# eldar/deepcut-cnn

Measured on AMD Instinct MI355X. Metric: images/sec, DeeperCut ResNet-152 FCN forward (prob+loc_pred+next_pred), whole node, higher is better.
Workload: dtype f32

## Files before the change

deepcut-cnn_amd/csrc/kernels.h:

```cpp
#pragma once
#include <cstddef>
#include <cstdint>
#include <string>

namespace dc {

constexpr int kMaxTaps = 32;

void dc_magic(unsigned d, unsigned (&mg)[2]);

enum ElemKind { kElemF32 = 0, kElemF16 = 1, kElemBF16 = 2 };
inline int elem_kind_size(int kind) { return kind == kElemF32 ? 4 : 2; }
inline const char* elem_kind_name(int kind) { return kind == kElemF16 ? "f16" : kind == kElemBF16 ? "bf16" : "f32"; }

constexpr int kMaxClasses = 4;
struct ConvClass {
  int nty, ntx, dy0, ddy, x0, ddx, Ktot, x_bias;
  int OH, OW, M;
  int tiles_m;
  unsigned div_ohw[2];
  unsigned div_ow[2];
  long w_off;
  long y_off;
};
// ... 20 lines not shown
  int end[8][kMaxProblems];
  ConvProblem prob[kMaxProblems];
};

struct ConvGemmParams {
  int esize;
  const void* x;
  long x_img_stride;
  int x_row_stride;
  int x_rows;
  int x_rowlen;
  int sy, sx;
  int nty, ntx;
  int dy0, ddy;
  int x0, ddx;
  int klen;
  int x_bias;
  const void* w;
  int Ktot;
  int NB, OH, OW;
  int M;
  int Cout;
  void* y;
  long y_img_stride;
  int y_row_stride;
  int y_pix_stride;
  const void* resid;
  const float* scale;
  const float* shift;
  int relu;
  int sigmoid_ch;
  int xcd_on;
  int xcd_lgx;
  int tiles_m;
  unsigned div_rw[2][2];
  unsigned div_ohw[2];
  unsigned div_ow[2];
  unsigned div_tn[2];
  int tiles_n;
  long long* dbg;
  int w_TY, w_TX, w_NBY, w_NBX, w_nblk;
  unsigned w_div_nblk[2], w_div_nbyx[2], w_div_dd[2], w_div_d[2], w_div_nbx[2];
  int wide_epi;
  int vec_epi;
  int dense_x;
  int dense_y;
  int ncls;
  int mc_lgx;
  ConvClass cls[kMaxClasses];
  int nprob;
  int ekind;
};
struct ConvMultiArgs {
  ConvGemmParams p;
  ConvMultiTable t;
};
static_assert(sizeof(ConvMultiArgs) <= 4096, "HIP kernel arguments are limited to 4 KB");

struct ConvVariant {
  const char* name;
  int BM, BN, WR, WC, WK;
};
int conv_num_variants();
const ConvVariant& conv_variant(int i);
int conv_variant_bk(int i);
int conv_variant_esize(int i);
constexpr int kBf16Variant0 = 2000;
int conv_num_bf16_variants();
inline bool is_bf16_variant(int v) { return v >= kBf16Variant0 && v < kBf16Variant0 + conv_num_bf16_variants(); }
int conv_variant_ekind(int v);
bool conv_variant_exists(int v);
const int* conv_variants_of(int ekind, int* count);
int conv_variant_by_name(const char* name);
bool conv_variant_multiclass(int i);
long conv_grid(const ConvGemmParams& p, int variant);
int launch_conv_gemm(const ConvGemmParams& p, int variant, void* stream);
long prepare_conv_multi(ConvGemmParams& p, ConvMultiTable& table, int nprob, int variant);
bool conv_variant_multiproblem(int i);
int launch_conv_multi(const ConvMultiArgs& a, int variant, long grid, void* stream);

bool wino_eligible(const ConvGemmParams& p);
bool wino_same3x3(const ConvGemmParams& p);
ConvGemmParams wino_launch_params(const ConvGemmParams& p, long grid, int bty, int btx, int blocks_per_wg);
long wino_grid(const ConvGemmParams& p);
size_t wino_packed_floats(int Cout, int Cin);
void wino_pack_filters(const float* g, int Cout, int Cin, float* out);
bool wino_half_eligible(const ConvGemmParams& p);
long wino_half_grid(const ConvGemmParams& p);
size_t wino_half_packed_elems(int Cout, int Cin);
void wino_half_pack_filters(const float* g, int Cout, int Cin, bool rowscale, float* out, float* row_scale);
int launch_wino_half(const ConvGemmParams& p, void* stream);
bool stream1x1_eligible(const ConvGemmParams& p);
long stream1x1_grid(const ConvGemmParams& p);
size_t stream1x1_packed_elems(int Cout, int K);
void stream1x1_pack_filters(const float* g, int Cout, int K, float* out);
int launch_stream1x1(const ConvGemmParams& p, void* stream);
bool stream1x1f_eligible(const ConvGemmParams& p);
long stream1x1f_grid(const ConvGemmParams& p);
size_t stream1x1f_packed_elems(int Cout, int K);
void stream1x1f_pack_filters(const float* g, int Cout, int K, float* out);
int launch_stream1x1f(const ConvGemmParams& p, void* stream);
bool stem_ws_eligible(const ConvGemmParams& p);
long stem_ws_grid(const ConvGemmParams& p);
size_t stem_ws_packed_elems();
void stem_ws_pack_filters(const float* rowtap, float* out);
int launch_stem_ws(const ConvGemmParams& p, void* stream);
bool stem7x7_eligible(const ConvGemmParams& p);
long stem7x7_grid(const ConvGemmParams& p);
size_t stem7x7_packed_elems();
void stem7x7_pack_filters(const float* g, int C, float* out);
int launch_stem7x7(const ConvGemmParams& p, void* stream);
long stream1x1_prepare_multi(const ConvGemmParams& p, const ConvMultiTable& tb, int nprob);
int launch_stream1x1_multi(const ConvMultiArgs& a, void* stream);

constexpr int kWinoVariant = 1000;
constexpr int kWinoVariant16 = 1001;
constexpr int kWinoHalf = 1002;
constexpr int kStreamHalf = 1003;
constexpr int kStemHalf = 1004;
constexpr int kStreamFloat = 1005;
constexpr int kStemFloat = 1006;
constexpr int kFormVariant0 = kWinoVariant, kNumForms = 7;
enum FormGeometry { kForm3x3, kForm1x1, kFormStem };
struct ConvForm {
  int variant;
  const char *name, *label;
  int ekind, geometry, waves;
  const char* const* timing_slots;
  bool (*eligible)(const ConvGemmParams& p);
  long (*grid)(const ConvGemmParams& p);
  int (*launch)(const ConvGemmParams& p, void* stream);
  bool own_scale;
  bool merges;
  long (*prepare_multi)(const ConvGemmParams& p, const ConvMultiTable& tb, int nprob);
  int (*launch_multi)(const ConvMultiArgs& a, void* stream);
  int sibling;
  const char* env;
};
const ConvForm* conv_form(int variant);

const char* variant_name(int v);
int variant_by_name(const char* name);
std::string variant_kernel_label(int v);
long variant_grid(const ConvGemmParams& p, int v);
int launch_conv(const ConvGemmParams& p, int v, void* stream);


int launch_maxpool(const void* x, void* y, int ekind, int NB, int H, int W, int C, int OH, int OW, int k, int s,
                   int pad, void* stream);

int launch_eltwise(const void* x, const void* z, const float* a, const float* b, void* y, int ekind, long total, int C,
                   int relu, int sigmoid, void* stream);

int launch_crop(const void* x, void* y, int ekind, int NB, int H, int W, int C, int oh, int ow, int OH, int OW,
                void* stream);

int launch_nchw_to_nhwc(const float* src, void* dst, int ekind, int NB, int C, int H, int W, int CP, void* stream);
int launch_nhwc_to_nchw(const void* src, void* dst, int ekind, int NB, int C, int H, int W, int CP, int c0,
                        void* stream, int dst_esize = 4);
int launch_f32_to_f16(const float* src, void* dst, long n, void* stream);
int launch_f32_to_bf16(const float* src, void* dst, long n, void* stream);

int launch_part_select(const void* prob, int pcp, int pc0, const void* loc, int lcp, int lc0, int ekind, int NB, int H, int W, int J, float thr,
                       int radius, double scale, int max_det, unsigned long long* spill, int* counts, double* out, void* stream);
int launch_pairwise_decode(const void* next, int ncp, int nc0, int ekind, int NB, int H, int W, int E, double scale, int ndet,
                           const int* det , const double* mean, const double* stdev, double* out,
                           void* stream);

struct ImagePrepParams {
  const unsigned char* src;
  int n, h, w;
  int out_h, out_w;
  int use_h, use_w;
  const int* x_bounds;
  const int* x_coeffs;
  int x_ksize;
  const int* y_bounds;
  const int* y_coeffs;
  int y_ksize;
  unsigned char* tmp;
  int row0, rows;
  void* dst;
  int dst_ekind, dst_cp;
  float mean[3];
};
int launch_image_prep(const ImagePrepParams& p, void* stream);

struct BoxPrepItem {
  int x0, y0, h, w;
  int use_h, use_w;
  const int* x_bounds;
  const int* x_coeffs;
  const int* y_bounds;
  const int* y_coeffs;
  int x_ksize, y_ksize;
};
struct BoxPrepParams {
  const unsigned char* src;
  int img_h, img_w;
  int n;
  int out_h, out_w;
  const BoxPrepItem* items;
  void* dst;
  int dst_ekind, dst_cp;
  float mean[3];
};
int launch_box_prep(const BoxPrepParams& p, void* stream);

int launch_pose_decode(const void* prob, int pcp, int pc0, const void* loc, int lcp, int lc0, int ekind, int NB, int H,
                       int W, int J, double scale, double* out, void* stream);
struct PoseDecodeItem {
  double scale, dx, dy;
  int rows, cols;
};
int launch_pose_decode_items(const void* prob, int pcp, int pc0, const void* loc, int lcp, int lc0, int ekind, int NB, int H,
                             int W, int J, const PoseDecodeItem* items, double* out, void* stream);

}
```

deepcut-cnn_amd/csrc/kernels.hip:

```cpp
#include <hip/hip_runtime.h>

#include <algorithm>
#include <cstdlib>
#include <cstring>
#include <type_traits>
#include <vector>

#include "kernel_prims.h"
#include "kernels.h"

namespace dc {


#define DC_KARG_TOUCH(n0, n1, n2, n3, n4)                                                                                  \
  unsigned n0, n1, n2, n3, n4;                                                                                             \
  {                                                                                                                        \
    const auto* ka_ = __builtin_amdgcn_kernarg_segment_ptr();                                                              \
    asm volatile("s_load_dword %0, %5, 0x0\n\ts_load_dword %1, %5, 0x40\n\ts_load_dword %2, %5, 0x80\n\ts_load_dword %3, %5, 0xc0\n\t" \
                 "s_load_dword %4, %5, 0x100"                                                                              \
                 : "=&s"(n0), "=&s"(n1), "=&s"(n2), "=&s"(n3), "=&s"(n4)                                                     \
                 : "s"(ka_));                                                                                              \
  }
#define DC_KARG_HOLD(n0, n1, n2, n3, n4) asm volatile("" ::"s"(n0), "s"(n1), "s"(n2), "s"(n3), "s"(n4))
static_assert(sizeof(ConvGemmParams) >= 0x140, "DC_KARG_TOUCH reads five 64-byte lines of the argument block");
// ... 1221 lines not shown
    const long g = f->prepare_multi ? f->prepare_multi(p, tb, nprob) : -1;
    if (g > 0) p.nprob = nprob, p.ncls = 0;
    return g;
  }
  if (!dc_variant_ok(variant) || nprob < 1 || nprob > kMaxProblems) return -1;
  const VariantEntry& e = entry_of(variant);
  if (!e.kernel_mp || p.esize != e.esize || (p.ekind == kElemBF16) != is_bf16_variant(variant) || p.klen % e.BK != 0) return -1;
  const long es = p.esize;
  const long tn = (p.Cout + e.v.BN - 1) / e.v.BN;
  bool vec = true;
  double atot = 0;
  long w_lo = 0, w_hi = 0;
  int rows[kMaxProblems];
  for (int c = 0; c < nprob; ++c) {
    ConvProblem& q = tb.prob[c];
    const int ntaps = q.nty * q.ntx;
    if (ntaps < 1 || ntaps > kMaxTaps || q.Ktot != ntaps * p.klen || q.M <= 0 || q.NB <= 0) return -1;
    if (!images_fit(es, q.NB, q.x_img_stride, q.y_img_stride)) return -1;
    if ((q.resid != nullptr) != (tb.prob[0].resid != nullptr)) return -1;
    q.x_bias = tap_bias(q, q.x_row_stride);
    set_m_tiles(q, e.v.BM);
    rows[c] = q.tiles_m;
    q.dense_x = dense_x_of(q, p);
    q.dense_y = dense_y_of(q);
    vec = vec && out_vec16(q, es);
    w_lo = std::min(w_lo, q.w_off);
    w_hi = std::max(w_hi, q.w_off + (long)p.Cout * q.Ktot);
    atot += (double)es * q.M * (double)p.klen * q.nty;
  }
  const double wtot = (double)es * (double)(w_hi - w_lo);
  if (wtot >= k2GiB) return -1;
  p.nprob = nprob;
  p.ncls = 0;
  set_epi(p, vec);
  p.dense_x = p.dense_y = 0;
  p.xcd_on = 0;
  p.tiles_n = (int)tn;
  dc_magic((unsigned)tn, p.div_tn);
  const long blk = mc_xcd_grid(p, rows, nprob, tn, wtot, atot);
  if (blk <= 0 || blk > 0x7fffffffL) return -1;
  {
    const int lgx = p.mc_lgx, lgy = 3 - lgx;
    const unsigned w0 = (unsigned)(tn >> lgx);
    dc_magic(std::max(w0, 1u), p.div_rw[0]);
    dc_magic(w0 + 1, p.div_rw[1]);
    for (int qy = 0; qy < 8; ++qy) {
      int run = 0;
      for (int c = 0; c < kMaxProblems; ++c) {
        if (c < nprob && qy < (8 >> lgx)) {
          run += (int)((((long)tb.prob[c].tiles_m * (qy + 1)) >> lgy) - (((long)tb.prob[c].tiles_m * qy) >> lgy));
          tb.end[qy][c] = run;
        } else {
          tb.end[qy][c] = 0x7fffffff;
        }
      }
    }
  }
  return blk;
}

int launch_conv_multi(const ConvMultiArgs& a, int variant, long grid, void* stream) {
  if (const ConvForm* f = conv_form(variant)) return f->launch_multi ? f->launch_multi(a, stream) : (int)hipErrorInvalidValue;
  if (!dc_variant_ok(variant) || !entry_of(variant).kernel_mp || a.p.nprob < 1 || grid <= 0) return (int)hipErrorInvalidValue;
  const VariantEntry& e = entry_of(variant);
  const int nt = e.v.WR * e.v.WC * e.v.WK * 64;
  hipLaunchKernelGGL(e.kernel_mp, dim3((unsigned)grid), dim3(nt), 0, (hipStream_t)stream, a);
  return (int)hipGetLastError();
}

namespace {
constexpr int WBTY = 4, WBTX = 8, WBN = 16, WKC = 32;
constexpr int WRH = 2 * WBTY + 2, WRW = 2 * WBTX + 2;
constexpr int WPSTR = WKC + 4;
constexpr int WPITCH = 672;
constexpr int WSTAGE = WRH * WPITCH + 8;
constexpr int WNTH = 512;
static_assert(WPITCH >= WRW * WPSTR && (2 * WPITCH) % 64 == 0 && WPSTR == 36, "conflict-free ds_read_b128 layout (see above)");
static_assert(WPITCH % 4 == 0 && WPSTR % 4 == 0 && WSTAGE % 4 == 0, "16-byte units");
__device__ __forceinline__ int wino_rowbase(int row) { return row * WPITCH; }
__device__ __forceinline__ f32x2 wlo(f32x4 v) { return __builtin_shufflevector(v, v, 0, 1); }
__device__ __forceinline__ f32x2 whi(f32x4 v) { return __builtin_shufflevector(v, v, 2, 3); }
}

template <int NG>
__global__ __launch_bounds__(WNTH * NG, 4) void wino_f23_kernel(const ConvGemmParams p) {
  constexpr int NTH = WNTH * NG;
  constexpr int WNLD = (WRH * WRW * (WKC / 4) + NTH - 1) / NTH;
  const long long t_entry = (long long)__builtin_amdgcn_s_memrealtime();
  DC_KARG_TOUCH(ka0, ka1, ka2, ka3, ka4);
  __shared__ __attribute__((aligned(16))) float stage[3][WSTAGE];
  float (*part)[4][2][2][4][64] = reinterpret_cast<float (*)[4][2][2][4][64]>(&stage[0][0]);
  static_assert(sizeof(float) * NG * 4 * 2 * 2 * 4 * 64 <= sizeof(stage), "partials must fit in the staging ring");
  static_assert(2 * sizeof(stage) <= 160 * 1024, "two workgroups per CU");
  const int t = threadIdx.x, lane = t & 63, wave = t >> 6;
  auto stamp = [&](int slot) {
    if (p.dbg && lane == 0) {
      long long* d = p.dbg + ((long)blockIdx.x * (8 * NG) + wave) * 12;
      d[slot] = (long long)__builtin_readcyclecounter();
      if (slot == 0) d[8] = t_entry, d[10] = (long long)__builtin_amdgcn_s_memrealtime();
      if (slot == 7) d[9] = (long long)__builtin_amdgcn_s_memrealtime();
    }
  };
  stamp(0);
  const int C = p.klen, H = p.x_rows, W = p.x_rowlen / p.klen;
  const int d = p.ddy;
  const int NBY = p.w_NBY, NBX = p.w_NBX;
  const int nblk = p.w_nblk;
  int lb = blockIdx.x;
  if (p.xcd_on) {
    const int g8 = gridDim.x >> 3, r8 = gridDim.x & 7, q = blockIdx.x & 7;
    lb = q * g8 + min(q, r8) + (blockIdx.x >> 3);
  }
  const int nt = dc_fastdiv(lb, p.w_div_nblk), blk = lb - nt * nblk;
  const int nph = dc_fastdiv(blk, p.w_div_nbyx), brem = blk - nph * (NBY * NBX);
  const int n = dc_fastdiv(nph, p.w_div_dd), ph = nph - n * (d * d);
  const int phy = dc_fastdiv(ph, p.w_div_d), phx = ph - phy * d;
  const int by = dc_fastdiv(brem, p.w_div_nbx), bx = brem - by * NBX;
  const int oy0 = 2 * WBTY * by - 1, ox0 = 2 * WBTX * bx - 1;
  DC_KARG_HOLD(ka0, ka1, ka2, ka3, ka4);
  const int kg = lane >> 4;
  const int grp = NG == 1 ? 0 : __builtin_amdgcn_readfirstlane(wave >> 3);
  const int i = wave & 3, tf = (wave >> 2) & 1;
  const int ra = i == 0 ? 0 : (i == 2 ? 2 : 1), rb = i == 0 ? 2 : (i == 1 ? 2 : (i == 2 ? 1 : 3));
  const float sb = i == 1 ? 1.f : -1.f;
  const __amdgpu_buffer_rsrc_t xr = dc_rsrc(reinterpret_cast<const float*>(p.x) + (long)n * p.x_img_stride, 0x7fffffffu);
  const __amdgpu_buffer_rsrc_t ur = dc_rsrc(p.w, 0x7fffffffu);
  unsigned gofs[WNLD];
  int sofs[WNLD];
#pragma unroll
  for (int q = 0; q < WNLD; ++q) {
    const int e = t + q * NTH;
    const int pix = e / (WKC / 4), cq = e % (WKC / 4);
    const int py = pix / WRW, px = pix % WRW;
    const int iy = phy + d * (oy0 + py), ix = phx + d * (ox0 + px);
    const bool ok = pix < WRH * WRW && oy0 + py >= 0 && ox0 + px >= 0 && iy < H && ix < W;
    gofs[q] = ok ? (unsigned)(iy * p.x_row_stride + ix * C + cq * 4) * 4u : kOOB;
    sofs[q] = (pix < WRH * WRW ? wino_rowbase(py) + px * WPSTR + cq * 4 : WSTAGE - 8 + (t & 1) * 4) >> 2;
  }
  const int r = (lane & 15) >> 3, c = lane & 7;
  const int ofs_a = wino_rowbase(2 * (2 * tf + r) + ra) + 2 * c * WPSTR + kg * 4;
  const int ofs_b = wino_rowbase(2 * (2 * tf + r) + rb) + 2 * c * WPSTR + kg * 4;
  f32x4 acc[4];
#pragma unroll
  for (int j = 0; j < 4; ++j) acc[j] = f32x4{0.f, 0.f, 0.f, 0.f};
  const unsigned uvo = ((unsigned)((nt * 4 + i) * (C / 16)) * (4 * 64 * 4) + (unsigned)lane * 4u) * 4u;
  f32x4 g[WNLD], b[2][4], da[4], db[4];
  auto gload = [&](int K) {
#pragma unroll
    for (int q = 0; q < WNLD; ++q) g[q] = dc_bload4(xr, gofs[q], (unsigned)(K * WKC * 4));
  };
  auto sstore = [&](int buf) {
#pragma unroll
    for (int q = 0; q < WNLD; ++q) reinterpret_cast<f32x4*>(&stage[buf][0])[sofs[q]] = g[q];
  };
  auto bload = [&](int slot, int k16) {
#pragma unroll
    for (int j = 0; j < 4; ++j) b[slot][j] = dc_bload4(ur, uvo + (unsigned)j * 1024u, (unsigned)k16 * 4096u);
  };
  auto lread = [&](int buf, int h) {
#pragma unroll
    for (int c4 = 0; c4 < 4; ++c4) {
      da[c4] = *reinterpret_cast<const f32x4*>(&stage[buf][ofs_a + c4 * WPSTR + h * 16]);
      db[c4] = *reinterpret_cast<const f32x4*>(&stage[buf][ofs_b + c4 * WPSTR + h * 16]);
    }
  };
  auto compute = [&](int bslot) {
    f32x2 tl[4], th[4];
    const f32x2 sb2 = {sb, sb};
#pragma unroll
    for (int c4 = 0; c4 < 4; ++c4) {
      tl[c4] = wlo(da[c4]) + sb2 * wlo(db[c4]);
      th[c4] = whi(da[c4]) + sb2 * whi(db[c4]);
    }
    f32x2 vl[4], vh[4];
    vl[0] = tl[0] - tl[2], vh[0] = th[0] - th[2];
    vl[1] = tl[1] + tl[2], vh[1] = th[1] + th[2];
    vl[2] = tl[2] - tl[1], vh[2] = th[2] - th[1];
    vl[3] = tl[1] - tl[3], vh[3] = th[1] - th[3];
#pragma unroll
    for (int j = 0; j < 4; ++j) acc[j] = __builtin_amdgcn_mfma_f32_16x16x4f32(vl[j][0], b[bslot][j][0], acc[j], 0, 0, 0);
#pragma unroll
    for (int j = 0; j < 4; ++j) acc[j] = __builtin_amdgcn_mfma_f32_16x16x4f32(vl[j][1], b[bslot][j][1], acc[j], 0, 0, 0);
#pragma unroll
    for (int j = 0; j < 4; ++j) acc[j] = __builtin_amdgcn_mfma_f32_16x16x4f32(vh[j][0], b[bslot][j][2], acc[j], 0, 0, 0);
#pragma unroll
    for (int j = 0; j < 4; ++j) acc[j] = __builtin_amdgcn_mfma_f32_16x16x4f32(vh[j][1], b[bslot][j][3], acc[j], 0, 0, 0);
  };
  const int NS = C / WKC;
  const int co = nt * WBN + (lane & 15);
  const float sc = p.scale ? p.scale[co] : 1.f, sh = p.shift ? p.shift[co] : 0.f;
  stamp(1);
  f32x4 g1[WNLD];
  gload(0);
  bload(0, grp);
  if (NS > 1) {
#pragma unroll
    for (int q = 0; q < WNLD; ++q) g1[q] = dc_bload4(xr, gofs[q], (unsigned)(WKC * 4));
  }
  stamp(2);
  sstore(0);
  if (NS > 2) gload(2);
  if (NS > 1) {
#pragma unroll
    for (int q = 0; q < WNLD; ++q) reinterpret_cast<f32x4*>(&stage[1][0])[sofs[q]] = g1[q];
  }
  stamp(3);
  if constexpr (NG == 1) {
    auto step = [&](int K, auto u_tag) {
      constexpr int U = decltype(u_tag)::value;
      __syncthreads();
      lread(U, 0);
      bload(1, 2 * K + 1);
      compute(0);
      if (K + 2 < NS) sstore((U + 2) % 3);
      lread(U, 1);
      bload(0, 2 * K + 2 < 2 * NS ? 2 * K + 2 : 0);
      compute(1);
      if (K + 3 < NS) gload(K + 3);
    };
    for (int K0 = 0; K0 < NS; K0 += 3) {
      step(K0, std::integral_constant<int, 0>{});
      if (K0 + 1 < NS) step(K0 + 1, std::integral_constant<int, 1>{});
      if (K0 + 2 < NS) step(K0 + 2, std::integral_constant<int, 2>{});
    }
  } else {
    auto step = [&](int K, auto u_tag, auto s_tag) {
      constexpr int U = decltype(u_tag)::value, S = decltype(s_tag)::value;
      __syncthreads();
      lread(U, grp);
      bload(S ^ 1, K + 1 < NS ? 2 * (K + 1) + grp : 0);
      compute(S);
      if (K + 2 < NS) sstore((U + 2) % 3);
      if (K + 3 < NS) gload(K + 3);
    };
    for (int K0 = 0; K0 < NS; K0 += 6) {
      step(K0, std::integral_constant<int, 0>{}, std::integral_constant<int, 0>{});
      if (K0 + 1 < NS) step(K0 + 1, std::integral_constant<int, 1>{}, std::integral_constant<int, 1>{});
      if (K0 + 2 < NS) step(K0 + 2, std::integral_constant<int, 2>{}, std::integral_constant<int, 0>{});
      if (K0 + 3 < NS) step(K0 + 3, std::integral_constant<int, 0>{}, std::integral_constant<int, 1>{});
      if (K0 + 4 < NS) step(K0 + 4, std::integral_constant<int, 1>{}, std::integral_constant<int, 0>{});
      if (K0 + 5 < NS) step(K0 + 5, std::integral_constant<int, 2>{}, std::integral_constant<int, 1>{});
    }
  }
  stamp(4);
  __syncthreads();
#pragma unroll
  for (int r4 = 0; r4 < 4; ++r4) {
    part[grp][i][0][tf][r4][lane] = acc[0][r4] + acc[1][r4] + acc[2][r4];
    part[grp][i][1][tf][r4][lane] = acc[1][r4] - acc[2][r4] - acc[3][r4];
  }
  __syncthreads();
  stamp(5);
  const int a = (wave >> 1) & 1, bq = wave & 1;
  float* yb = reinterpret_cast<float*>(p.y);
  const float* rbp = reinterpret_cast<const float*>(p.resid);
  stamp(6);
#pragma unroll
  for (int rr = 0; rr < 4 / NG; ++rr) {
    const int r4 = NG == 1 ? rr : 2 * grp + rr;
    float p0 = part[0][0][bq][tf][r4][lane], p1 = part[0][1][bq][tf][r4][lane], p2 = part[0][2][bq][tf][r4][lane], p3 = part[0][3][bq][tf][r4][lane];
    if constexpr (NG == 2) {
      p0 += part[NG - 1][0][bq][tf][r4][lane], p1 += part[NG - 1][1][bq][tf][r4][lane];
      p2 += part[NG - 1][2][bq][tf][r4][lane], p3 += part[NG - 1][3][bq][tf][r4][lane];
    }
    float v = a == 0 ? p0 + p1 + p2 : p1 - p2 - p3;
    const int q = 4 * (lane >> 4) + r4;
    const int ty = by * WBTY + 2 * tf + (q >> 3), tx = bx * WBTX + (q & 7);
    const int oy = phy + d * (2 * ty + a), ox = phx + d * (2 * tx + bq);
    if (oy < p.OH && ox < p.OW) {
      const long off = (long)n * p.y_img_stride + (long)oy * p.y_row_stride + (long)ox * p.y_pix_stride + co;
      v = v * sc + sh;
      if (rbp) v += rbp[off];
      if (p.relu) v = fmaxf(v, 0.f);
      yb[off] = v;
    }
  }
  stamp(7);
}

bool wino_same3x3(const ConvGemmParams& p) {
  const int d = p.ddy;
  if (p.nty != 3 || p.ntx != 3 || p.sy != 1 || d < 1 || d > 4 || p.dy0 != -d) return false;
  const int C = p.klen;
  if (C <= 0) return false;
  if (p.sx != C || p.ddx != d * C || p.x0 != -d * C) return false;
  if (p.x_rowlen % C != 0 || p.x_row_stride != p.x_rowlen) return false;
  return p.OH == p.x_rows && p.OW == p.x_rowlen / C;
}

ConvGemmParams wino_launch_params(const ConvGemmParams& p, long grid, int bty, int btx, int blocks_per_wg) {
  ConvGemmParams q = p;
  q.xcd_on = xcd_map_on() && grid >= 16;
  const int d = p.ddy;
  q.w_TY = ((p.OH + d - 1) / d + 1) / 2, q.w_TX = ((p.OW + d - 1) / d + 1) / 2;
  q.w_NBY = (q.w_TY + bty - 1) / bty, q.w_NBX = (q.w_TX + btx - 1) / btx;
  q.w_nblk = p.NB * d * d * q.w_NBY * q.w_NBX;
  dc_magic((unsigned)((q.w_nblk + blocks_per_wg - 1) / blocks_per_wg), q.w_div_nblk);
  dc_magic((unsigned)(q.w_NBY * q.w_NBX), q.w_div_nbyx);
  dc_magic((unsigned)(d * d), q.w_div_dd);
  dc_magic((unsigned)d, q.w_div_d);
  dc_magic((unsigned)q.w_NBX, q.w_div_nbx);
  return q;
}

bool wino_eligible(const ConvGemmParams& p) {
  if (p.esize != 4 || !wino_same3x3(p)) return false;
  const int C = p.klen;
  if (C % WKC != 0 || p.Cout % WBN != 0 || p.sigmoid_ch != 0) return false;
  if ((long long)p.x_rows * p.x_row_stride * 4 >= 0x7fffffffLL || (long long)wino_packed_floats(p.Cout, C) * 4 >= 0x7fffffffLL) return false;
  return true;
}

long wino_grid(const ConvGemmParams& p) {
  const int d = p.ddy;
  const int TY = ((p.OH + d - 1) / d + 1) / 2, TX = ((p.OW + d - 1) / d + 1) / 2;
  return (long)p.NB * d * d * ((TY + WBTY - 1) / WBTY) * ((TX + WBTX - 1) / WBTX) * (p.Cout / WBN);
}

size_t wino_packed_floats(int Cout, int Cin) { return (size_t)16 * Cout * Cin; }

void wino_pack_filters(const float* g, int Cout, int Cin, float* out) {
  static const double G[4][3] = {{1, 0, 0}, {.5, .5, .5}, {.5, -.5, .5}, {0, 0, 1}};
  for (int co = 0; co < Cout; ++co)
    for (int ci = 0; ci < Cin; ++ci) {
      const float* w = g + ((size_t)co * Cin + ci) * 9;
      double tmp[4][3], U[4][4];
      for (int a = 0; a < 4; ++a)
        for (int b = 0; b < 3; ++b) tmp[a][b] = G[a][0] * w[b] + G[a][1] * w[3 + b] + G[a][2] * w[6 + b];
      for (int a = 0; a < 4; ++a)
        for (int b = 0; b < 4; ++b) U[a][b] = tmp[a][0] * G[b][0] + tmp[a][1] * G[b][1] + tmp[a][2] * G[b][2];
      const int nt = co / 16, col = co % 16, k16 = ci / 16, kg = (ci % 16) / 4, s = ci % 4;
      const int lane = kg * 16 + col;
      for (int i = 0; i < 4; ++i)
        for (int j = 0; j < 4; ++j)
          out[(((((size_t)nt * 4 + i) * (Cin / 16) + k16) * 4 + j) * 64 + lane) * 4 + s] = (float)U[i][j];
    }
}

template <int NG>
static int launch_wino_f23(const ConvGemmParams& p, void* stream) {
  if (p.esize != 4 || !wino_eligible(p)) return (int)hipErrorInvalidValue;
  const long grid = wino_grid(p);
  if (grid <= 0) return 0;
  if (grid > 0x7fffffffL) return (int)hipErrorInvalidValue;
  hipLaunchKernelGGL(wino_f23_kernel<NG>, dim3((unsigned)grid), dim3(NG * WNTH), 0, (hipStream_t)stream, wino_launch_params(p, grid, WBTY, WBTX, 1));
  return (int)hipGetLastError();
}

static const char* const kWinoSlots[7] = {"index setup", "first loads issued", "two stages in LDS", "K loop", "partials to LDS + barrier",
                                          "inverse transform + epilogue constants", "shortcut + stores"};
static const char* const kStreamSlots[7] = {"prologue requests issued", "first stage + filters landed", "the first D steps", "the other steps",
                                            "drain", "-", "exit"};
static constexpr ConvForm kForms[kNumForms] = {
    {kWinoVariant, "wino_f23", "wino_f23<4x8x16>", kElemF32, kForm3x3, 8, kWinoSlots, wino_eligible, wino_grid, launch_wino_f23<1>,
     false, false, nullptr, nullptr, kWinoVariant16, "DC_WINOGRAD"},
    {kWinoVariant16, "wino_f23_w16", "wino_f23<4x8x16_w16>", kElemF32, kForm3x3, 16, kWinoSlots, wino_eligible, wino_grid, launch_wino_f23<2>,
     false, false, nullptr, nullptr, kWinoVariant, "DC_WINOGRAD"},
    {kWinoHalf, "wino_h23", "wino_h23<2x4x8x64>", kElemF16, kForm3x3, 8, kWinoSlots, wino_half_eligible, wino_half_grid, launch_wino_half,
     true, true, nullptr, nullptr, -1, "DC_WINOGRAD"},
    {kStreamHalf, "ws1x1", "ws1x1<32xN>", kElemF16, kForm1x1, 4, kStreamSlots, stream1x1_eligible, stream1x1_grid, launch_stream1x1,
     false, true, stream1x1_prepare_multi, launch_stream1x1_multi, -1, "DC_STREAM1X1"},
    {kStemHalf, "stem7x7", "stem7x7<8x64>", kElemF16, kFormStem, 4, kWinoSlots, stem7x7_eligible, stem7x7_grid, launch_stem7x7,
     false, false, nullptr, nullptr, -1, "DC_STEM"},
    {kStreamFloat, "ws1x1f", "ws1x1f<16xN>", kElemF32, kForm1x1, 4, kStreamSlots, stream1x1f_eligible, stream1x1f_grid, launch_stream1x1f,
     false, true, nullptr, nullptr, -1, "DC_STREAM1X1"},
    {kStemFloat, "ws7x7f", "ws7x7f<16x64>", kElemF32, kFormStem, 4, kStreamSlots, stem_ws_eligible, stem_ws_grid, launch_stem_ws,
     false, true, nullptr, nullptr, -1, "DC_STEM"},
};

static constexpr bool forms_in_variant_order() {
  for (int i = 0; i < kNumForms; ++i)
    if (kForms[i].variant != kFormVariant0 + i) return false;
  return true;
}
static_assert(forms_in_variant_order(), "row i of kForms is variant kFormVariant0 + i");

const ConvForm* conv_form(int variant) {
  return variant >= kFormVariant0 && variant < kFormVariant0 + kNumForms ? &kForms[variant - kFormVariant0] : nullptr;
}

const char* variant_name(int v) {
  const ConvForm* f = conv_form(v);
  return f ? f->name : conv_variant(v).name;
}
int variant_by_name(const char* name) {
  for (const ConvForm& f : kForms)
    if (std::strcmp(name, f.name) == 0) return f.variant;
  return conv_variant_by_name(name);
}
std::string variant_kernel_label(int v) {
  const ConvForm* f = conv_form(v);
  return f ? std::string(f->label) : std::string("conv_gemm<") + conv_variant(v).name + ">";
}
long variant_grid(const ConvGemmParams& p, int v) {
  const ConvForm* f = conv_form(v);
  return f ? f->grid(p) : conv_grid(p, v);
}
int launch_conv(const ConvGemmParams& p, int v, void* stream) {
  const ConvForm* f = conv_form(v);
  return f ? f->launch(p, stream) : launch_conv_gemm(p, v, stream);
}

template <typename F>
static int dc_by_kind(int ekind, F&& f) {
  if (ekind == kElemF16) return f((_Float16*)nullptr);
  if (ekind == kElemBF16) return f((__bf16*)nullptr);
  return f((float*)nullptr);
}
template <typename T>
__device__ __forceinline__ T dc_lowest() {
  if constexpr (std::is_same_v<T, float>) return (T)-3.402823466e+38f;
  else if constexpr (std::is_same_v<T, _Float16>) return (T)-65504.f;
  else return __builtin_bit_cast(T, (unsigned short)0xff7fu);
}

template <typename T>
__global__ __launch_bounds__(256) void maxpool_kernel(const T* __restrict__ x, T* __restrict__ y, int NB, int H, int W,
                                                      int C, int OH, int OW, int k, int s, int pad) {
  constexpr int V = 16 / sizeof(T);
  typedef T vec_t __attribute__((ext_vector_type(V)));
  const int cvn = C / V;
  long idx = (long)blockIdx.x * blockDim.x + threadIdx.x;
  long total = (long)NB * OH * OW * cvn;
  if (idx >= total) return;
  int cv = (int)(idx % cvn);
  long pix = idx / cvn;
  int ox = (int)(pix % OW);
  long t2 = pix / OW;
  int oy = (int)(t2 % OH);
  int n = (int)(t2 / OH);
  int hs = oy * s - pad, ws = ox * s - pad;
  int he = min(hs + k, H), we = min(ws + k, W);
  hs = max(hs, 0);
  ws = max(ws, 0);
  vec_t m;
#pragma unroll
  for (int q = 0; q < V; ++q) m[q] = dc_lowest<T>();
  for (int iy = hs; iy < he; ++iy)
    for (int ix = ws; ix < we; ++ix) {
      vec_t v = *reinterpret_cast<const vec_t*>(x + (((long)n * H + iy) * W + ix) * C + cv * V);
#pragma unroll
      for (int q = 0; q < V; ++q) m[q] = v[q] > m[q] ? v[q] : m[q];
    }
  *reinterpret_cast<vec_t*>(y + (((long)n * OH + oy) * OW + ox) * C + cv * V) = m;
}

template <typename T>
__global__ __launch_bounds__(256) void maxpool_scalar_kernel(const T* __restrict__ x, T* __restrict__ y, int NB, int H,
                                                             int W, int C, int OH, int OW, int k, int s, int pad) {
  long idx = (long)blockIdx.x * blockDim.x + threadIdx.x;
  long total = (long)NB * OH * OW * C;
  if (idx >= total) return;
  int c = (int)(idx % C);
  long pix = idx / C;
  int ox = (int)(pix % OW);
  long t2 = pix / OW;
  int oy = (int)(t2 % OH);
  int n = (int)(t2 / OH);
  int hs = oy * s - pad, ws = ox * s - pad;
  int he = min(hs + k, H), we = min(ws + k, W);
  hs = max(hs, 0);
  ws = max(ws, 0);
  float m = -3.402823466e+38f;
  for (int iy = hs; iy < he; ++iy)
    for (int ix = ws; ix < we; ++ix) {
      float v = (float)x[(((long)n * H + iy) * W + ix) * C + c];
      m = v > m ? v : m;
    }
  y[idx] = (T)m;
}

template <typename T>
static int launch_maxpool_t(const void* x, void* y, int NB, int H, int W, int C, int OH, int OW, int k, int s, int pad,
                            void* stream) {
  constexpr int V = 16 / sizeof(T);
// ... 585 lines not shown
```

deepcut-cnn_amd/csrc/net_image.cpp:

```cpp
#include "net_internal.h"

namespace dc {

#pragma clang fp contract(off)
ResampleTable::~ResampleTable() {
  dev_free(dev_bounds);
  dev_free(dev_coeffs);
}

void resample_coeffs(int in_size, int out_size, int& ksize, std::vector<int>& bounds, std::vector<int>& coeffs) {
  const int kPrecisionBits = 32 - 8 - 2;
  double filterscale, scale;
  filterscale = scale = (double)in_size / out_size;
  if (filterscale < 1.0) filterscale = 1.0;
  const double support = 1.0 * filterscale;
  ksize = (int)std::ceil(support) * 2 + 1;
  bounds.assign((size_t)out_size * 2, 0);
  coeffs.assign((size_t)out_size * ksize, 0);
  std::vector<double> k(ksize);
  for (int xx = 0; xx < out_size; ++xx) {
    const double center = 0.0 + (xx + 0.5) * scale;
    double ww = 0.0;
    const double ss = 1.0 / filterscale;
    int xmin = (int)(center - support + 0.5);
// ... 300 lines not shown
  if (s.head == UNINITIALIZED) throw DcError(DC_EINVAL, std::string("'") + blob_name + "': run forward() first");
  if (s.shape.size() != 4) throw DcError(DC_ESHAPE, std::string("'") + blob_name + "' is not a 4-D map");
  MapRef r{};
  if (s.view_of >= 0) {
    Storage& b = *storages[s.view_of];
    r.ptr = b.dev, r.cp = b.cp(), r.c0 = s.view_c0, r.es = b.esize, r.ek = b.ekind;
  } else {
    if (s.head == HEAD_AT_CPU) sync_to_device(s);
    r.ptr = s.dev, r.cp = s.cp(), r.c0 = 0, r.es = s.esize, r.ek = s.ekind;
  }
  r.NB = s.dim(0), r.C = s.dim(1), r.H = s.dim(2), r.W = s.dim(3);
  return r;
}

void* Net::scratch(size_t bytes) {
  if (bytes > scratch_cap_) {
    dev_free(scratch_dev_);
    scratch_dev_ = nullptr;
    dev_alloc((void**)&scratch_dev_, bytes);
    scratch_cap_ = bytes;
  }
  return scratch_dev_;
}

void Net::detect_parts(double scale, float thr, int radius, int max_det, int* counts, double* dets) {
  if (Context::get().mode != DC_MODE_GPU) throw DcError(DC_ENOCPU, "detect_parts() in CPU mode");
  if (!(scale > 0) || !(thr >= 0.f) || radius < 0 || radius > 64 || max_det < 1 || max_det > 4096)
    throw DcError(DC_EINVAL, "detect_parts: scale > 0, threshold >= 0, 0 <= radius <= 64, 1 <= max_det <= 4096");
  ensure_device();
  const MapRef P = map_ref("prob"), L = map_ref("loc_pred");
  if (L.C != 2 * P.C || L.H != P.H || L.W != P.W || L.NB != P.NB || L.es != P.es)
    throw DcError(DC_ESHAPE, "detect_parts: loc_pred must have 2 channels per joint and the score map's size");
  const int lists = P.NB * P.C;
  const size_t cnt_b = ((size_t)lists * sizeof(int) + 255) / 256 * 256;
  const size_t spill_b = (size_t)lists * P.H * P.W * sizeof(unsigned long long);
  const size_t out_b = (size_t)lists * max_det * 5 * sizeof(double);
  unsigned char* base = (unsigned char*)scratch(cnt_b + spill_b + out_b);
  int* cnt = (int*)base;
  unsigned long long* spill = (unsigned long long*)(base + cnt_b);
  double* out = (double*)(base + cnt_b + spill_b);
  KCHECK(launch_part_select(P.ptr, P.cp, P.c0, L.ptr, L.cp, L.c0, P.ek, P.NB, P.H, P.W, P.C, thr, radius, scale, max_det, spill, cnt, out,
                            stream));
  HIPCHECK(hipMemcpyAsync(counts, cnt, (size_t)lists * sizeof(int), hipMemcpyDeviceToHost, (hipStream_t)stream));
  HIPCHECK(hipMemcpyAsync(dets, out, out_b, hipMemcpyDeviceToHost, (hipStream_t)stream));
  HIPCHECK(hipStreamSynchronize((hipStream_t)stream));
}

void Net::decode_pairwise(double scale, int ndet, const int* det, const double* mean, const double* stdev, double* out) {
  if (Context::get().mode != DC_MODE_GPU) throw DcError(DC_ENOCPU, "decode_pairwise() in CPU mode");
  if (!(scale > 0) || ndet < 0) throw DcError(DC_EINVAL, "decode_pairwise: scale > 0, ndet >= 0");
  if (ndet == 0) return;
  ensure_device();
  const MapRef N = map_ref("next_pred");
  if (N.C % 2) throw DcError(DC_ESHAPE, "decode_pairwise: next_pred must have 2 channels per regression edge");
  const int E = N.C / 2;
  const size_t det_b = ((size_t)ndet * 3 * sizeof(int) + 255) / 256 * 256, st_b = (size_t)E * 2 * sizeof(double);
  const size_t out_b = (size_t)ndet * E * 2 * sizeof(double);
  unsigned char* base = (unsigned char*)scratch(det_b + 2 * st_b + out_b);
  int* ddet = (int*)base;
  double* dmean = (double*)(base + det_b);
  double* dstd = dmean + (size_t)E * 2;
  double* dout = (double*)(base + det_b + 2 * st_b);
  HIPCHECK(hipMemcpyAsync(ddet, det, (size_t)ndet * 3 * sizeof(int), hipMemcpyHostToDevice, (hipStream_t)stream));
  if (mean) HIPCHECK(hipMemcpyAsync(dmean, mean, st_b, hipMemcpyHostToDevice, (hipStream_t)stream));
  if (stdev) HIPCHECK(hipMemcpyAsync(dstd, stdev, st_b, hipMemcpyHostToDevice, (hipStream_t)stream));
  KCHECK(launch_pairwise_decode(N.ptr, N.cp, N.c0, N.ek, N.NB, N.H, N.W, E, scale, ndet, ddet, mean ? dmean : nullptr,
                                stdev ? dstd : nullptr, dout, stream));
  HIPCHECK(hipMemcpyAsync(out, dout, out_b, hipMemcpyDeviceToHost, (hipStream_t)stream));
  HIPCHECK(hipStreamSynchronize((hipStream_t)stream));
}

std::string Net::plan_text() {
  ensure_plan();
  std::ostringstream os;
  os << "# plan for input";
  for (int d : plan_input_shape) os << " " << d;
  os << ": " << plan.size() << " launches, " << plan_flops / 1e9 << " GFLOP algorithmic, fuse=" << fuse
     << ", dtype=" << elem_kind_name(dtype) << "\n";
  for (size_t i = 0; i < plan.size(); ++i) {
    const Launch& l = plan[i];
    os << i << "\t" << l.kernel << "\t";
    if (l.kind == Launch::CONV)
      os << "M=" << l.cg.M << " N=" << l.cg.Cout << " K=" << l.cg.Ktot << " taps=" << l.cg.nty * l.cg.ntx
         << (l.cg.ncls > 1 ? " classes=" + std::to_string(l.cg.ncls) : std::string()) << " grid=" << l.grid
         << (l.in2 >= 0 ? " +resid" : "") << (l.relu ? " +relu" : "") << (l.cg.sigmoid_ch ? " +sigmoid" : "");
    os << "\t" << l.label << "\n";
  }
  return os.str();
}

std::string Net::profile_text(int iters) {
  if (Context::get().mode != DC_MODE_GPU) throw DcError(DC_ENOCPU, "profile in CPU mode");
  if (!plan_valid) throw DcError(DC_EINVAL, "profile_text: run forward() first");
  ensure_device();
  hipEvent_t e0, e1;
  HIPCHECK(hipEventCreate(&e0));
  HIPCHECK(hipEventCreate(&e1));
  std::ostringstream os;
  os << "idx\tkernel\tus\tGFLOP\tTFLOP/s\tgrid\tlabel\n";
  double total_us = 0;
  for (size_t i = 0; i < plan.size(); ++i) {
    const Launch& l = plan[i];
    run_launch(l, stream);
    HIPCHECK(hipEventRecord(e0, (hipStream_t)stream));
    for (int k = 0; k < iters; ++k) run_launch(l, stream);
    HIPCHECK(hipEventRecord(e1, (hipStream_t)stream));
    HIPCHECK(hipEventSynchronize(e1));
    float ms = 0;
    HIPCHECK(hipEventElapsedTime(&ms, e0, e1));
    double us = ms * 1000.0 / iters;
    total_us += us;
    char buf[512];
    std::snprintf(buf, sizeof buf, "%zu\t%s\t%.2f\t%.3f\t%.2f\t%ld\t%s\n", i, l.kernel.c_str(), us, l.flops / 1e9,
                  us > 0 ? l.flops / us / 1e6 : 0.0, l.grid, l.label.c_str());
    os << buf;
  }
  os << "# sum of per-launch times: " << total_us << " us\n";
  (void)hipEventDestroy(e0);
  (void)hipEventDestroy(e1);
  return os.str();
}


std::string Net::debug_info_text() {
  if (!plan_valid) throw DcError(DC_EINVAL, "debug_info: run forward() first");
  std::ostringstream os;
  char buf[384];
  auto mean_abs = [&](Storage& st) -> double {
    sync_to_host(st);
    const float* h = st.host_ptr();
    const size_t n = st.count();
    double a = 0;
    for (size_t i = 0; i < n; ++i) a += std::fabs((double)h[i]);
    return n ? a / (double)n : 0.0;
  };
  for (int b : inputs) {
    std::snprintf(buf, sizeof buf, "    [Forward] Input %s data: %g\n", blobs[b]->name.c_str(), mean_abs(*blobs[b]->st));
    os << buf;
  }
  std::vector<int> last_writer(blobs.size(), -1);
  for (size_t i = 0; i < layers.size(); ++i)
    for (int t : layers[i].tops) last_writer[t] = (int)i;
  for (size_t i = 0; i < layers.size(); ++i) {
    const LayerRec& L = layers[i];
    for (int t : L.tops) {
      Storage& st = *blobs[t]->st;
      if (last_writer[t] != (int)i) {
        std::snprintf(buf, sizeof buf, "    [Forward] Layer %s, top blob %s data: (in place: folded into layer %s)\n", L.name.c_str(),
                      blobs[t]->name.c_str(), layers[last_writer[t]].name.c_str());
      } else if (st.elided) {
        std::snprintf(buf, sizeof buf, "    [Forward] Layer %s, top blob %s data: (elided by fusion; DC_OPT_FUSE 0 materialises it)\n",
                      L.name.c_str(), blobs[t]->name.c_str());
      } else {
        std::snprintf(buf, sizeof buf, "    [Forward] Layer %s, top blob %s data: %g\n", L.name.c_str(), blobs[t]->name.c_str(), mean_abs(st));
      }
      os << buf;
    }
    for (size_t k = 0; k < L.params.size(); ++k) {
      Storage& st = *L.params[k]->st;
      const float* h = st.host_ptr();
      const size_t n = st.count();
      double a = 0;
      for (size_t q = 0; q < n; ++q) a += std::fabs((double)h[q]);
      const auto specs = L.def.subs("param");
      const std::string pname = k < specs.size() && !specs[k]->str("name").empty() ? specs[k]->str("name") : std::to_string(k);
      std::snprintf(buf, sizeof buf, "    [Forward] Layer %s, param blob %s data: %g\n", L.name.c_str(), pname.c_str(), n ? a / (double)n : 0.0);
      os << buf;
// ... 7 lines not shown
```

Baseline: 519.0.

## Widen Winograd F(2,3) kernel to 32 output channels per workgroup

Adds a wide variant of the single-group Winograd F(2,3) kernel in which each workgroup computes two 16-channel output slices. The transformed input tile is reused across both slices, and filter loads are interleaved with the MFMA chain. The wide form is used by default when the resulting grid is still at least 256 workgroups, with environment overrides. This cuts input-transform work and LDS traffic per output, at the cost of more accumulator registers, a smaller grid, and possibly lower occupancy.

```diff
diff --git a/deepcut-cnn_amd/csrc/kernels.h b/deepcut-cnn_amd/csrc/kernels.h
--- a/deepcut-cnn_amd/csrc/kernels.h
+++ b/deepcut-cnn_amd/csrc/kernels.h
@@ -126,6 +126,7 @@
 bool wino_eligible(const ConvGemmParams& p);
 bool wino_same3x3(const ConvGemmParams& p);
 ConvGemmParams wino_launch_params(const ConvGemmParams& p, long grid, int bty, int btx, int blocks_per_wg);
+int wino_width(const ConvGemmParams& p);
 long wino_grid(const ConvGemmParams& p);
 size_t wino_packed_floats(int Cout, int Cin);
 void wino_pack_filters(const float* g, int Cout, int Cin, float* out);
@@ -187,6 +188,7 @@
 int variant_by_name(const char* name);
 std::string variant_kernel_label(int v);
 long variant_grid(const ConvGemmParams& p, int v);
+std::string variant_plan_note(const ConvGemmParams& p, int v);
 int launch_conv(const ConvGemmParams& p, int v, void* stream);
 
 
diff --git a/deepcut-cnn_amd/csrc/kernels.hip b/deepcut-cnn_amd/csrc/kernels.hip
--- a/deepcut-cnn_amd/csrc/kernels.hip
+++ b/deepcut-cnn_amd/csrc/kernels.hip
@@ -1327,15 +1327,17 @@
 __device__ __forceinline__ f32x2 whi(f32x4 v) { return __builtin_shufflevector(v, v, 2, 3); }
 }
 
-template <int NG>
+template <int NG, int WN>
 __global__ __launch_bounds__(WNTH * NG, 4) void wino_f23_kernel(const ConvGemmParams p) {
+  static_assert(WN == WBN || (WN == 2 * WBN && NG == 1), "16 output channels per workgroup, or 32 on the 8-wave form");
   constexpr int NTH = WNTH * NG;
+  constexpr int NSL = WN / WBN;
   constexpr int WNLD = (WRH * WRW * (WKC / 4) + NTH - 1) / NTH;
   const long long t_entry = (long long)__builtin_amdgcn_s_memrealtime();
   DC_KARG_TOUCH(ka0, ka1, ka2, ka3, ka4);
   __shared__ __attribute__((aligned(16))) float stage[3][WSTAGE];
   float (*part)[4][2][2][4][64] = reinterpret_cast<float (*)[4][2][2][4][64]>(&stage[0][0]);
-  static_assert(sizeof(float) * NG * 4 * 2 * 2 * 4 * 64 <= sizeof(stage), "partials must fit in the staging ring");
+  static_assert(sizeof(float) * NG * NSL * 4 * 2 * 2 * 4 * 64 <= sizeof(stage), "partials must fit in the staging ring");
   static_assert(2 * sizeof(stage) <= 160 * 1024, "two workgroups per CU");
   const int t = threadIdx.x, lane = t & 63, wave = t >> 6;
   auto stamp = [&](int slot) {
@@ -1385,10 +1387,13 @@
   const int r = (lane & 15) >> 3, c = lane & 7;
   const int ofs_a = wino_rowbase(2 * (2 * tf + r) + ra) + 2 * c * WPSTR + kg * 4;
   const int ofs_b = wino_rowbase(2 * (2 * tf + r) + rb) + 2 * c * WPSTR + kg * 4;
-  f32x4 acc[4];
-#pragma unroll
-  for (int j = 0; j < 4; ++j) acc[j] = f32x4{0.f, 0.f, 0.f, 0.f};
-  const unsigned uvo = ((unsigned)((nt * 4 + i) * (C / 16)) * (4 * 64 * 4) + (unsigned)lane * 4u) * 4u;
+  f32x4 acc[NSL][4];
+#pragma unroll
+  for (int s = 0; s < NSL; ++s)
+#pragma unroll
+    for (int j = 0; j < 4; ++j) acc[s][j] = f32x4{0.f, 0.f, 0.f, 0.f};
+  const unsigned uvo = ((unsigned)((nt * NSL * 4 + i) * (C / 16)) * (4 * 64 * 4) + (unsigned)lane * 4u) * 4u;
+  const unsigned usl = (unsigned)C * 1024u;
   f32x4 g[WNLD], b[2][4], da[4], db[4];
   auto gload = [&](int K) {
 #pragma unroll
@@ -1409,7 +1414,8 @@
       db[c4] = *reinterpret_cast<const f32x4*>(&stage[buf][ofs_b + c4 * WPSTR + h * 16]);
     }
   };
-  auto compute = [&](int bslot) {
+  f32x2 vl[4], vh[4];
+  auto transform = [&]() {
     f32x2 tl[4], th[4];
     const f32x2 sb2 = {sb, sb};
 #pragma unroll
@@ -1417,27 +1423,61 @@
       tl[c4] = wlo(da[c4]) + sb2 * wlo(db[c4]);
       th[c4] = whi(da[c4]) + sb2 * whi(db[c4]);
     }
-    f32x2 vl[4], vh[4];
     vl[0] = tl[0] - tl[2], vh[0] = th[0] - th[2];
     vl[1] = tl[1] + tl[2], vh[1] = th[1] + th[2];
     vl[2] = tl[2] - tl[1], vh[2] = th[2] - th[1];
     vl[3] = tl[1] - tl[3], vh[3] = th[1] - th[3];
-#pragma unroll
-    for (int j = 0; j < 4; ++j) acc[j] = __builtin_amdgcn_mfma_f32_16x16x4f32(vl[j][0], b[bslot][j][0], acc[j], 0, 0, 0);
-#pragma unroll
-    for (int j = 0; j < 4; ++j) acc[j] = __builtin_amdgcn_mfma_f32_16x16x4f32(vl[j][1], b[bslot][j][1], acc[j], 0, 0, 0);
-#pragma unroll
-    for (int j = 0; j < 4; ++j) acc[j] = __builtin_amdgcn_mfma_f32_16x16x4f32(vh[j][0], b[bslot][j][2], acc[j], 0, 0, 0);
-#pragma unroll
-    for (int j = 0; j < 4; ++j) acc[j] = __builtin_amdgcn_mfma_f32_16x16x4f32(vh[j][1], b[bslot][j][3], acc[j], 0, 0, 0);
+  };
+  auto compute = [&](int bslot) {
+    transform();
+#pragma unroll
+    for (int j = 0; j < 4; ++j) acc[0][j] = __builtin_amdgcn_mfma_f32_16x16x4f32(vl[j][0], b[bslot][j][0], acc[0][j], 0, 0, 0);
+#pragma unroll
+    for (int j = 0; j < 4; ++j) acc[0][j] = __builtin_amdgcn_mfma_f32_16x16x4f32(vl[j][1], b[bslot][j][1], acc[0][j], 0, 0, 0);
+#pragma unroll
+    for (int j = 0; j < 4; ++j) acc[0][j] = __builtin_amdgcn_mfma_f32_16x16x4f32(vh[j][0], b[bslot][j][2], acc[0][j], 0, 0, 0);
+#pragma unroll
+    for (int j = 0; j < 4; ++j) acc[0][j] = __builtin_amdgcn_mfma_f32_16x16x4f32(vh[j][1], b[bslot][j][3], acc[0][j], 0, 0, 0);
+  };
+  auto compute2 = [&](int next) {
+    transform();
+#pragma unroll
+    for (int h = 0; h < 2; ++h) {
+#pragma unroll
+      for (int e = 0; e < 4; ++e) {
+        const f32x2 v0 = e < 2 ? vl[2 * h] : vh[2 * h], v1 = e < 2 ? vl[2 * h + 1] : vh[2 * h + 1];
+#pragma unroll
+        for (int s = 0; s < NSL; ++s) {
+          acc[s][2 * h] = __builtin_amdgcn_mfma_f32_16x16x4f32(v0[e & 1], b[s][2 * h][e], acc[s][2 * h], 0, 0, 0);
+          acc[s][2 * h + 1] = __builtin_amdgcn_mfma_f32_16x16x4f32(v1[e & 1], b[s][2 * h + 1][e], acc[s][2 * h + 1], 0, 0, 0);
+        }
+      }
+#pragma unroll
+      for (int s = 0; s < NSL; ++s)
+#pragma unroll
+        for (int j = 2 * h; j < 2 * h + 2; ++j) b[s][j] = dc_bload4(ur, uvo + (unsigned)j * 1024u, (unsigned)next * 4096u + (unsigned)s * usl);
+      if (h == 0) __builtin_amdgcn_sched_barrier(0);
+    }
   };
   const int NS = C / WKC;
-  const int co = nt * WBN + (lane & 15);
-  const float sc = p.scale ? p.scale[co] : 1.f, sh = p.shift ? p.shift[co] : 0.f;
+  const int co = nt * WN + (lane & 15);
+  float sc[NSL], sh[NSL];
+  auto epi_consts = [&]() {
+#pragma unroll
+    for (int s = 0; s < NSL; ++s) sc[s] = p.scale ? p.scale[co + s * WBN] : 1.f, sh[s] = p.shift ? p.shift[co + s * WBN] : 0.f;
+  };
+  if constexpr (NSL == 1) epi_consts();
   stamp(1);
   f32x4 g1[WNLD];
   gload(0);
-  bload(0, grp);
+  if constexpr (NSL == 1) {
+    bload(0, grp);
+  } else {
+#pragma unroll
+    for (int s = 0; s < NSL; ++s)
+#pragma unroll
+      for (int j = 0; j < 4; ++j) b[s][j] = dc_bload4(ur, uvo + (unsigned)j * 1024u, (unsigned)s * usl);
+  }
   if (NS > 1) {
 #pragma unroll
     for (int q = 0; q < WNLD; ++q) g1[q] = dc_bload4(xr, gofs[q], (unsigned)(WKC * 4));
@@ -1455,12 +1495,20 @@
       constexpr int U = decltype(u_tag)::value;
       __syncthreads();
       lread(U, 0);
-      bload(1, 2 * K + 1);
-      compute(0);
+      if constexpr (NSL == 1) {
+        bload(1, 2 * K + 1);
+        compute(0);
+      } else {
+        compute2(2 * K + 1);
+      }
       if (K + 2 < NS) sstore((U + 2) % 3);
       lread(U, 1);
-      bload(0, 2 * K + 2 < 2 * NS ? 2 * K + 2 : 0);
-      compute(1);
+      if constexpr (NSL == 1) {
+        bload(0, 2 * K + 2 < 2 * NS ? 2 * K + 2 : 0);
+        compute(1);
+      } else {
+        compute2(2 * K + 2 < 2 * NS ? 2 * K + 2 : 0);
+      }
       if (K + 3 < NS) gload(K + 3);
     };
     for (int K0 = 0; K0 < NS; K0 += 3) {
@@ -1488,12 +1536,15 @@
     }
   }
   stamp(4);
+  if constexpr (NSL > 1) epi_consts();
   __syncthreads();
 #pragma unroll
-  for (int r4 = 0; r4 < 4; ++r4) {
-    part[grp][i][0][tf][r4][lane] = acc[0][r4] + acc[1][r4] + acc[2][r4];
-    part[grp][i][1][tf][r4][lane] = acc[1][r4] - acc[2][r4] - acc[3][r4];
-  }
+  for (int s = 0; s < NSL; ++s)
+#pragma unroll
+    for (int r4 = 0; r4 < 4; ++r4) {
+      part[grp + s][i][0][tf][r4][lane] = acc[s][0][r4] + acc[s][1][r4] + acc[s][2][r4];
+      part[grp + s][i][1][tf][r4][lane] = acc[s][1][r4] - acc[s][2][r4] - acc[s][3][r4];
+    }
   __syncthreads();
   stamp(5);
   const int a = (wave >> 1) & 1, bq = wave & 1;
@@ -1501,9 +1552,10 @@
   const float* rbp = reinterpret_cast<const float*>(p.resid);
   stamp(6);
 #pragma unroll
-  for (int rr = 0; rr < 4 / NG; ++rr) {
+  for (int rs = 0; rs < NSL * 4 / NG; ++rs) {
+    const int s = NG == 1 ? rs >> 2 : 0, rr = rs & 3;
     const int r4 = NG == 1 ? rr : 2 * grp + rr;
-    float p0 = part[0][0][bq][tf][r4][lane], p1 = part[0][1][bq][tf][r4][lane], p2 = part[0][2][bq][tf][r4][lane], p3 = part[0][3][bq][tf][r4][lane];
+    float p0 = part[s][0][bq][tf][r4][lane], p1 = part[s][1][bq][tf][r4][lane], p2 = part[s][2][bq][tf][r4][lane], p3 = part[s][3][bq][tf][r4][lane];
     if constexpr (NG == 2) {
       p0 += part[NG - 1][0][bq][tf][r4][lane], p1 += part[NG - 1][1][bq][tf][r4][lane];
       p2 += part[NG - 1][2][bq][tf][r4][lane], p3 += part[NG - 1][3][bq][tf][r4][lane];
@@ -1513,8 +1565,8 @@
     const int ty = by * WBTY + 2 * tf + (q >> 3), tx = bx * WBTX + (q & 7);
     const int oy = phy + d * (2 * ty + a), ox = phx + d * (2 * tx + bq);
     if (oy < p.OH && ox < p.OW) {
-      const long off = (long)n * p.y_img_stride + (long)oy * p.y_row_stride + (long)ox * p.y_pix_stride + co;
-      v = v * sc + sh;
+      const long off = (long)n * p.y_img_stride + (long)oy * p.y_row_stride + (long)ox * p.y_pix_stride + co + s * WBN;
+      v = v * sc[s] + sh[s];
       if (rbp) v += rbp[off];
       if (p.relu) v = fmaxf(v, 0.f);
       yb[off] = v;
@@ -1556,11 +1608,24 @@
   return true;
 }
 
-long wino_grid(const ConvGemmParams& p) {
+static long wino_grid_at(const ConvGemmParams& p, int width);
+constexpr long kWinoWideMinGrid = 256;
+int wino_width(const ConvGemmParams& p) {
+  const char* e = getenv("DC_WINO_WIDTH");
+  const int want = e ? atoi(e) : 0;
+  if (p.Cout % (2 * WBN) != 0 || want == WBN) return WBN;
+  if (want == 2 * WBN) return 2 * WBN;
+  const char* g = getenv("DC_WINO_WIDTH_MIN_GRID");
+  return wino_grid_at(p, 2 * WBN) >= (g ? atol(g) : kWinoWideMinGrid) ? 2 * WBN : WBN;
+}
+
+static long wino_grid_at(const ConvGemmParams& p, int width) {
   const int d = p.ddy;
   const int TY = ((p.OH + d - 1) / d + 1) / 2, TX = ((p.OW + d - 1) / d + 1) / 2;
-  return (long)p.NB * d * d * ((TY + WBTY - 1) / WBTY) * ((TX + WBTX - 1) / WBTX) * (p.Cout / WBN);
-}
+  return (long)p.NB * d * d * ((TY + WBTY - 1) / WBTY) * ((TX + WBTX - 1) / WBTX) * (p.Cout / width);
+}
+long wino_grid(const ConvGemmParams& p) { return wino_grid_at(p, wino_width(p)); }
+static long wino_grid_w16(const ConvGemmParams& p) { return wino_grid_at(p, WBN); }
 
 size_t wino_packed_floats(int Cout, int Cin) { return (size_t)16 * Cout * Cin; }
 
@@ -1585,10 +1650,18 @@
 template <int NG>
 static int launch_wino_f23(const ConvGemmParams& p, void* stream) {
   if (p.esize != 4 || !wino_eligible(p)) return (int)hipErrorInvalidValue;
-  const long grid = wino_grid(p);
+  const int width = NG == 1 ? wino_width(p) : WBN;
+  const long grid = wino_grid_at(p, width);
   if (grid <= 0) return 0;
   if (grid > 0x7fffffffL) return (int)hipErrorInvalidValue;
-  hipLaunchKernelGGL(wino_f23_kernel<NG>, dim3((unsigned)grid), dim3(NG * WNTH), 0, (hipStream_t)stream, wino_launch_params(p, grid, WBTY, WBTX, 1));
+  const ConvGemmParams q = wino_launch_params(p, grid, WBTY, WBTX, 1);
+  if constexpr (NG == 1) {
+    if (width == 2 * WBN) {
+      hipLaunchKernelGGL((wino_f23_kernel<1, 2 * WBN>), dim3((unsigned)grid), dim3(WNTH), 0, (hipStream_t)stream, q);
+      return (int)hipGetLastError();
+    }
+  }
+  hipLaunchKernelGGL((wino_f23_kernel<NG, WBN>), dim3((unsigned)grid), dim3(NG * WNTH), 0, (hipStream_t)stream, q);
   return (int)hipGetLastError();
 }
 
@@ -1599,7 +1672,7 @@
 static constexpr ConvForm kForms[kNumForms] = {
     {kWinoVariant, "wino_f23", "wino_f23<4x8x16>", kElemF32, kForm3x3, 8, kWinoSlots, wino_eligible, wino_grid, launch_wino_f23<1>,
      false, false, nullptr, nullptr, kWinoVariant16, "DC_WINOGRAD"},
-    {kWinoVariant16, "wino_f23_w16", "wino_f23<4x8x16_w16>", kElemF32, kForm3x3, 16, kWinoSlots, wino_eligible, wino_grid, launch_wino_f23<2>,
+    {kWinoVariant16, "wino_f23_w16", "wino_f23<4x8x16_w16>", kElemF32, kForm3x3, 16, kWinoSlots, wino_eligible, wino_grid_w16, launch_wino_f23<2>,
      false, false, nullptr, nullptr, kWinoVariant, "DC_WINOGRAD"},
     {kWinoHalf, "wino_h23", "wino_h23<2x4x8x64>", kElemF16, kForm3x3, 8, kWinoSlots, wino_half_eligible, wino_half_grid, launch_wino_half,
      true, true, nullptr, nullptr, -1, "DC_WINOGRAD"},
@@ -1636,6 +1709,9 @@
 std::string variant_kernel_label(int v) {
   const ConvForm* f = conv_form(v);
   return f ? std::string(f->label) : std::string("conv_gemm<") + conv_variant(v).name + ">";
+}
+std::string variant_plan_note(const ConvGemmParams& p, int v) {
+  return v == kWinoVariant ? " width=" + std::to_string(wino_width(p)) : std::string();
 }
 long variant_grid(const ConvGemmParams& p, int v) {
   const ConvForm* f = conv_form(v);
diff --git a/deepcut-cnn_amd/csrc/net_image.cpp b/deepcut-cnn_amd/csrc/net_image.cpp
--- a/deepcut-cnn_amd/csrc/net_image.cpp
+++ b/deepcut-cnn_amd/csrc/net_image.cpp
@@ -406,7 +406,7 @@
     os << i << "\t" << l.kernel << "\t";
     if (l.kind == Launch::CONV)
       os << "M=" << l.cg.M << " N=" << l.cg.Cout << " K=" << l.cg.Ktot << " taps=" << l.cg.nty * l.cg.ntx
-         << (l.cg.ncls > 1 ? " classes=" + std::to_string(l.cg.ncls) : std::string()) << " grid=" << l.grid
+         << (l.cg.ncls > 1 ? " classes=" + std::to_string(l.cg.ncls) : std::string()) << " grid=" << l.grid << variant_plan_note(l.cg, l.variant)
          << (l.in2 >= 0 ? " +resid" : "") << (l.relu ? " +relu" : "") << (l.cg.sigmoid_ch ? " +sigmoid" : "");
     os << "\t" << l.label << "\n";
   }
```

Result: no change. 523.9, median of 6 (+1.0%).
